# AdamClixby/Modulate

Measured on AMD Instinct MI355X. Metric: GB/s encrypt+decrypt over synthetic .ark parts; % HBM peak at 1/2/4/8 GPU, higher is better.
Workload: dtype u8

## Files before the change

include/modgpu_testing.h:

```cpp
#ifndef MODGPU_TESTING_H
#define MODGPU_TESTING_H

#include <stdint.h>

#ifdef __cplusplus
extern "C" {
#endif

int modgpu_time_cycle_device(void *dev_buf, uint64_t n, int32_t key, uint64_t stream_off,
                             int device, void *hip_stream, int iters, float *ms_per_launch);

int modgpu_time_cycle_device_to(void *dev_dst, const void *dev_src, uint64_t n, int32_t key, uint64_t stream_off,
                                int device, void *hip_stream, int iters, float *ms_per_launch);

int modgpu_time_rekey_device_to(void *dev_dst, const void *dev_src, uint64_t n, int32_t key_from, uint64_t off_from, int32_t key_to,
                                uint64_t off_to, int device, void *hip_stream, int iters, float *ms_per_launch);
int modgpu_time_cycle_table_device(const void *dev_entries, uint64_t n_entries, void *dev_workspace,
                                   uint64_t workspace_bytes, int device, void *hip_stream, int iters, float *ms_per_call);
int modgpu_time_rekey_table_device(const void *dev_entries, uint64_t n_entries, void *dev_workspace,
                                   uint64_t workspace_bytes, int device, void *hip_stream, int iters, float *ms_per_call);

int modgpu_time_verify_device(const void *dev_expect, const void *dev_src, uint64_t n, int32_t key, uint64_t stream_off,
                              void *dev_result, int device, void *hip_stream, int iters, float *ms_per_call);
int modgpu_time_digest_device(void *dev_dst, const void *dev_src, uint64_t n, int32_t key, uint64_t stream_off, void *dev_result,
// ... 53 lines not shown

int modgpu_cycle_scalar_host_isa(uint8_t *host_buf, uint64_t n, int32_t key, uint64_t stream_off, const char *isa);

int modgpu_numa_probe(const char *sysfs_root, const char *bdf, int *node, int *cpus, int max_cpus);

int modgpu_host_alloc_on_node(void **host_ptr, uint64_t n, int node);

void modgpu_queue_stats(uint64_t out[6]);

const char *modgpu_kernel_source_hash(void);
const char *modgpu_feed_kernel_source_hash(void);
const char *modgpu_to_kernel_source_hash(void);
const char *modgpu_xfer_kernel_source_hash(void);
const char *modgpu_rekey_kernel_source_hash(void);
const char *modgpu_table_kernel_source_hash(void);
const char *modgpu_rekey_table_kernel_source_hash(void);
const char *modgpu_verify_kernel_source_hash(void);
const char *modgpu_verify_table_kernel_source_hash(void);
const char *modgpu_rekey_verify_kernel_source_hash(void);
const char *modgpu_keep_kernel_source_hash(void);
const char *modgpu_rekey_verify_table_kernel_source_hash(void);
const char *modgpu_rekey_move_table_kernel_source_hash(void);
int modgpu_keep_policy(uint64_t bytes, uint32_t *mask, uint32_t *run);

int modgpu_testing_hooks(void);


void modgpu_debug_set_queue_ring(uint32_t lines);

void modgpu_debug_set_to_form(int form);

void modgpu_debug_set_rekey_form(int shape);

void modgpu_debug_set_table_grid(uint32_t grid);

void modgpu_debug_set_rekey_table_grid(uint32_t grid);

void modgpu_debug_set_move_grid(uint32_t grid);

void modgpu_debug_set_move_table_grid(uint32_t grid);

void modgpu_debug_set_verify_form(int grid);
void modgpu_debug_set_digest_grid(int grid);

void modgpu_debug_set_verify_table_grid(uint32_t grid);

void modgpu_debug_set_rekey_verify_table_grid(uint32_t grid);

void modgpu_debug_set_digest_table_grid(uint32_t grid);

void modgpu_debug_set_cycle_digest_table_grid(uint32_t grid);

void modgpu_debug_set_rekey_digest_table_grid(uint32_t grid);

void modgpu_debug_set_keep(uint64_t min_bytes, uint32_t mask, uint32_t run);

void modgpu_debug_set_xfer_form(int form);

void modgpu_debug_set_helpers(int mode);

void modgpu_debug_set_batch(int mode);

void modgpu_debug_set_launch(int variant, uint32_t grid_cap);

enum { MODGPU_TUNABLE_ZEROCOPY_BYTES = 0, MODGPU_TUNABLE_RING = 1, MODGPU_TUNABLE_SPLIT = 2, MODGPU_TUNABLE_CHUNK_MIN_BYTES = 3,
       MODGPU_TUNABLE_RAMP_BYTES = 4, MODGPU_TUNABLE_LANES = 5, MODGPU_TUNABLE_NTCOPY = 6,
       MODGPU_TUNABLE_FILE_SCHED = 7,
       MODGPU_TUNABLE_FEED = 8,
       MODGPU_TUNABLE_FEED_CHUNK_BYTES = 9,
       MODGPU_TUNABLE_FEED_PATIENCE_MS = 10,
       MODGPU_TUNABLE_FILE_FEED = 11,
       MODGPU_TUNABLE_XFER_LIST_MOST_BYTES = 12  };
void modgpu_debug_set_host_tunable(int which, uint64_t value);

void modgpu_debug_set_gpu_node(int node);

void modgpu_debug_set_pcie_grid(uint32_t cap);

// ... 22 lines not shown
```

modulate_amd/__init__.py:

```python
from .capi import (
    ModGpuError, lib, lib_path, device_count, cycle_host, cycle_device, hdr_decrypt_host,
    hdr_encrypt_host, cycle_parts_host, cycle_parts_device, cycle_batch_device, cycle_host_split, debug_set_batch, cycle_file, cycle_file_to_host, cycle_host_to_file, DeviceBuffer, time_cycle_device, state_at, jump_table,
    KEY_PS3, KEY_PS4, MAGIC_PS3, MAGIC_PS4, as_int32, EXPORTS, TESTING_EXPORTS, cycle_scalar_host, cycle_auto_host,
    path_stats, gpu_required, last_launch, debug_set_launch, debug_set_pinned_mode, debug_set_staged_mode, kernel_source_hash, feed_kernel_source_hash, prepare, host_tunables, debug_inject_failures, debug_inject_failure_at, debug_injection_armed, debug_hold_slots, debug_forbid_worker_threads, debug_set_pcie_grid, debug_set_gpu_node, debug_set_host_tunable, HOST_TUNABLES, STAGE_FILL, STAGE_LAUNCH, STAGE_SYNC, STAGE_DRAIN, STAGE_AFTER_DRAIN, STAGE_STALL, INJECT_PIECE_LAST, INJECT_PIECE_MIDDLE, PinnedBuffer, host_register, host_unregister,
    DEBUG_EXPORTS, FLAVOURS, testing_flavour, use_testing_flavour, active_flavour, debug_set_queue_ring, debug_set_helpers, queue_stats, testing_hooks, min_gpu_bytes,
    cycle_device_to, cycle_batch_device_to, time_cycle_device_to, to_kernel_source_hash, debug_set_to_form, TO_FORMS,
    rekey_device_to, rekey_batch_device_to, time_rekey_device_to, rekey_kernel_source_hash, debug_set_rekey_form, REKEY_FORMS,
    rekey_move_device, move_workspace_bytes, move_status, debug_set_move_grid,
    rekey_move_table_device, rekey_move_table_workspace_bytes, rekey_move_table_validate, rekey_move_table_status, compaction_table,
    rekey_move_table_kernel_source_hash, debug_set_move_table_grid,
    rekey_relayout_table_device, rekey_relayout_table_validate, relayout_table, splice_moves,
    cycle_table_device, time_cycle_table_device, table, table_workspace_bytes, table_status, table_validate, table_kernel_source_hash,
    debug_set_table_grid, TableEntry, TABLE_DTYPE,
    rekey_table_device, time_rekey_table_device, rekey_table, rekey_table_workspace_bytes, rekey_table_validate,
    rekey_table_kernel_source_hash, debug_set_rekey_table_grid, RekeyTableEntry, REKEY_TABLE_DTYPE,
    verify_device, verify_batch_device, verify_results, time_verify_device, verify_kernel_source_hash, debug_set_verify_form,
    VERIFY_RESULT_DTYPE, VERIFY_NONE,
    digest_device, digest_batch_device, digest_results, digest_adler32, time_digest_device, debug_set_digest_grid, DIGEST_RESULT_DTYPE,
    verify_table_device, verify_table_summary, verify_table_workspace_bytes, time_verify_table_device, verify_table_kernel_source_hash,
    debug_set_verify_table_grid, VERIFY_TABLE_SUMMARY_DTYPE,
    digest_table_device, digest_table_workspace_bytes, time_digest_table_device, debug_set_digest_table_grid,
    cycle_digest_table_device, cycle_digest_table_workspace_bytes, time_cycle_digest_table_device, debug_set_cycle_digest_table_grid,
    DIGEST_OUTPUT, DIGEST_INPUT,
    rekey_digest_table_device, rekey_digest_table_workspace_bytes, time_rekey_digest_table_device, debug_set_rekey_digest_table_grid,
    DIGEST_PLAIN,
    digest_check_device, digest_check_result, digest_check_bits_bytes, time_digest_check_device, DIGEST_CHECK_SUMMARY_DTYPE,
    verify_rekey_table_device, verify_rekey_table_workspace_bytes, time_verify_rekey_table_device, rekey_verify_table_kernel_source_hash,
    debug_set_rekey_verify_table_grid,
    verify_rekey_device, verify_rekey_batch_device, time_verify_rekey_device, rekey_verify_kernel_source_hash,
    keep_kernel_source_hash, keep_policy, debug_set_keep, KEEP_OFF,
    cycle_host_to_device, cycle_device_to_host, cycle_host_to_device_list, cycle_device_to_host_list, cycle_host_to_device_list_digest, cycle_device_to_host_list_digest, cycle_file_to_device, cycle_device_to_file, xfer_kernel_source_hash, debug_set_xfer_form, XFER_FORMS,
    host_loop_isa, cycle_scalar_host_isa, device_numa_node, numa_probe, host_policy, host_policy_engine, host_trace, host_trace_read, host_pool_stats, host_chunking, HOST_TRACE_KINDS,
)
```

modulate_amd/capi.py:

```python
import contextlib
import ctypes
import os

import numpy as np

_HERE = os.path.dirname(os.path.abspath(__file__))

KEY_PS3 = 0xC64EED30
KEY_PS4 = 0x90CFC0AB
MAGIC_PS3 = 0xC64EED30
MAGIC_PS4 = 0x6F303F55

_u64, _i32, _int, _vp = ctypes.c_uint64, ctypes.c_int32, ctypes.c_int, ctypes.c_void_p
EXPORTS = {
    "modgpu_abi_version": (_int, []),
    "modgpu_device_count": (_int, []),
    "modgpu_last_error": (ctypes.c_char_p, []),
    "modgpu_cycle_device": (_int, [_vp, _u64, _i32, _u64, _int, _vp]),
    "modgpu_cycle_host": (_int, [_vp, _u64, _i32, _u64, _int]),
    "modgpu_hdr_decrypt_host": (_int, [_vp, _u64, _int]),
    "modgpu_hdr_encrypt_host": (_int, [_vp, _u64, _int, _int]),
    "modgpu_cycle_parts_host": (_int, [ctypes.POINTER(_vp), ctypes.POINTER(_u64), _int, _i32, _int]),
    "modgpu_cycle_parts_device": (_int, [ctypes.POINTER(_vp), ctypes.POINTER(_u64), ctypes.POINTER(_int), _int, _i32]),
    "modgpu_cycle_host_split": (_int, [_vp, _u64, _i32, _u64, _int]),
# ... 150 lines not shown
    "modgpu_time_cycle_device_to": (_int, [_vp, _vp, _u64, _i32, _u64, _int, _vp, _int, ctypes.POINTER(ctypes.c_float)]),
    "modgpu_to_kernel_source_hash": (ctypes.c_char_p, []),
    "modgpu_xfer_kernel_source_hash": (ctypes.c_char_p, []),
    "modgpu_time_rekey_device_to": (_int, [_vp, _vp, _u64, _i32, _u64, _i32, _u64, _int, _vp, _int, ctypes.POINTER(ctypes.c_float)]),
    "modgpu_rekey_kernel_source_hash": (ctypes.c_char_p, []),
    "modgpu_time_cycle_table_device": (_int, [_vp, _u64, _vp, _u64, _int, _vp, _int, ctypes.POINTER(ctypes.c_float)]),
    "modgpu_table_kernel_source_hash": (ctypes.c_char_p, []),
    "modgpu_time_rekey_table_device": (_int, [_vp, _u64, _vp, _u64, _int, _vp, _int, ctypes.POINTER(ctypes.c_float)]),
    "modgpu_rekey_table_kernel_source_hash": (ctypes.c_char_p, []),
    "modgpu_time_verify_device": (_int, [_vp, _vp, _u64, _i32, _u64, _vp, _int, _vp, _int, ctypes.POINTER(ctypes.c_float)]),
    "modgpu_verify_kernel_source_hash": (ctypes.c_char_p, []),
    "modgpu_time_verify_table_device": (_int, [_vp, _u64, _vp, _vp, _u64, _int, _vp, _int, ctypes.POINTER(ctypes.c_float)]),
    "modgpu_verify_table_kernel_source_hash": (ctypes.c_char_p, []),
    "modgpu_time_digest_table_device": (_int, [_vp, _u64, _vp, _vp, _u64, _int, _vp, _int, ctypes.POINTER(ctypes.c_float)]),
    "modgpu_time_cycle_digest_table_device": (_int, [_vp, _u64, _vp, ctypes.c_uint32, _vp, _u64, _int, _vp, _int, ctypes.POINTER(ctypes.c_float)]),
    "modgpu_time_rekey_digest_table_device": (_int, [_vp, _u64, _vp, ctypes.c_uint32, _vp, _u64, _int, _vp, _int, ctypes.POINTER(ctypes.c_float)]),
    "modgpu_time_verify_rekey_device": (_int, [_vp, _vp, _u64, _i32, _u64, _i32, _u64, _vp, _int, _vp, _int, ctypes.POINTER(ctypes.c_float)]),
    "modgpu_rekey_verify_kernel_source_hash": (ctypes.c_char_p, []),
    "modgpu_keep_kernel_source_hash": (ctypes.c_char_p, []),
    "modgpu_time_verify_rekey_table_device": (_int, [_vp, _u64, _vp, _vp, _u64, _int, _vp, _int, ctypes.POINTER(ctypes.c_float)]),
    "modgpu_rekey_verify_table_kernel_source_hash": (ctypes.c_char_p, []),
    "modgpu_rekey_move_table_kernel_source_hash": (ctypes.c_char_p, []),
    "modgpu_keep_policy": (_int, [_u64, ctypes.POINTER(ctypes.c_uint32), ctypes.POINTER(ctypes.c_uint32)]),
    "modgpu_time_digest_device": (_int, [_vp, _vp, _u64, _i32, _u64, _vp, _int, _vp, _int, ctypes.POINTER(ctypes.c_float)]),
    "modgpu_time_digest_check_device": (_int, [_vp, _vp, _u64, _vp, _vp, _vp, _int, _vp, _int, ctypes.POINTER(ctypes.c_float)]),
}
DEBUG_EXPORTS = {
    "modgpu_debug_set_launch": (None, [_int, ctypes.c_uint32]),
    "modgpu_debug_set_pinned_mode": (None, [_int]),
    "modgpu_debug_set_staged_mode": (None, [_int]),
    "modgpu_debug_set_queue_ring": (None, [ctypes.c_uint32]),
    "modgpu_debug_set_helpers": (None, [_int]),
    "modgpu_debug_set_batch": (None, [_int]),
    "modgpu_debug_set_pcie_grid": (None, [ctypes.c_uint32]),
    "modgpu_debug_set_gpu_node": (None, [_int]),
    "modgpu_debug_set_host_tunable": (None, [_int, _u64]),
    "modgpu_debug_inject_failures": (None, [_int]),
    "modgpu_debug_inject_failure_at": (None, [ctypes.c_int64, _int]),
    "modgpu_debug_injection_armed": (_int, []),
    "modgpu_debug_hold_slots": (_int, [_int, _int]),
    "modgpu_debug_forbid_worker_threads": (None, [_int]),
    "modgpu_debug_set_to_form": (None, [_int]),
    "modgpu_debug_set_xfer_form": (None, [_int]),
    "modgpu_debug_set_rekey_form": (None, [_int]),
    "modgpu_debug_set_table_grid": (None, [ctypes.c_uint32]),
    "modgpu_debug_set_rekey_table_grid": (None, [ctypes.c_uint32]),
    "modgpu_debug_set_move_grid": (None, [ctypes.c_uint32]),
    "modgpu_debug_set_move_table_grid": (None, [ctypes.c_uint32]),
    "modgpu_debug_set_verify_form": (None, [_int]),
    "modgpu_debug_set_verify_table_grid": (None, [ctypes.c_uint32]),
    "modgpu_debug_set_rekey_verify_table_grid": (None, [ctypes.c_uint32]),
    "modgpu_debug_set_digest_table_grid": (None, [ctypes.c_uint32]),
    "modgpu_debug_set_cycle_digest_table_grid": (None, [ctypes.c_uint32]),
    "modgpu_debug_set_rekey_digest_table_grid": (None, [ctypes.c_uint32]),
    "modgpu_debug_set_keep": (None, [_u64, ctypes.c_uint32, ctypes.c_uint32]),
    "modgpu_debug_set_digest_grid": (None, [_int]),
}


class ModGpuError(RuntimeError):
    def __init__(self, code, text):
        super().__init__(f"modgpu error {code}: {text}")
        self.code = code


FLAVOURS = {"shipped": "libmodgpu.so", "testing": "libmodgpu_testing.so"}


def lib_path(flavour="shipped"):
    return os.environ.get("MODGPU_LIB") or os.path.join(_HERE, FLAVOURS[flavour])


_libs = {}
_active = "shipped"


def _load(flavour):
    if flavour not in _libs:
# ... 782 lines not shown

def time_verify_rekey_device(expect, src, n, key_from, key_to, result, off_from=0, off_to=0, device=-1, stream=None, iters=2):
    return _time_call("modgpu_time_verify_rekey_device", (_vp(_dev_addr(expect)), _vp(_dev_addr(src)), n, as_int32(key_from), off_from,
                                                          as_int32(key_to), off_to, _vp(_dev_addr(result))), device, stream, iters)


def keep_kernel_source_hash():
    return lib().modgpu_keep_kernel_source_hash().decode()


KEEP_OFF = (1 << 64) - 1


def keep_policy(nbytes):
    mask, run = ctypes.c_uint32(), ctypes.c_uint32()
    route = lib().modgpu_keep_policy(nbytes, ctypes.byref(mask), ctypes.byref(run))
    return bool(route), mask.value, run.value


def debug_set_keep(min_bytes=0, mask=0, run=0):
    _debug_lib().modgpu_debug_set_keep(min_bytes, mask, run)


def rekey_verify_kernel_source_hash():
    return lib().modgpu_rekey_verify_kernel_source_hash().decode()


def verify_table_workspace_bytes(n_entries):
    return lib().modgpu_verify_table_workspace_bytes(n_entries)


def verify_table_summary(workspace, device=-1):
    out = np.zeros(1, dtype=VERIFY_TABLE_SUMMARY_DTYPE)
    _check(lib().modgpu_verify_table_summary(_vp(_dev_addr(workspace)), device, _vp(out.ctypes.data)))
    first = int(out["first_bad_entry"][0])
    return {"mismatches": int(out["mismatches"][0]), "first_bad_entry": None if first == VERIFY_NONE else first, "entries": int(out["entries"][0])}


def verify_table_device(entries, results=None, workspace=None, device=-1, stream=None, *, n=None):
    return _table_call("modgpu_verify_table_device", entries, TABLE_DTYPE, n, workspace, verify_table_workspace_bytes, device, stream,
                       "the device refused verify table entry {}; no result was written", fetch=verify_results, results=results,
                       empty=_no_verify_results)


def time_verify_table_device(entries, n, results, workspace, device=-1, stream=None, iters=2):
    ws_bytes = workspace.nbytes if isinstance(workspace, DeviceBuffer) else verify_table_workspace_bytes(n)
# ... 470 lines not shown
```

modulate_amd/csrc/cycle_keep_kernel.h:

```cpp
#pragma once
#include <hip/hip_runtime.h>
#include <cstdint>

#include "cycle_kernel.h"

struct CycleKeepArgs : CycleQueueArgs {
    uint32_t keep_mask;
    uint32_t keep_run;
};
uint32_t modgpu_keep_chunk_bytes();
uint32_t modgpu_keep_block();
const char *modgpu_keep_kernel_name();
hipError_t modgpu_launch_cycle_keep(const CycleKeepArgs &a, uint32_t grid, hipStream_t stream);
```

modulate_amd/csrc/cycle_keep_kernel.hip:

```cpp
#include <hip/hip_runtime.h>
#include <cstdint>

#include "cycle_kernel_impl.h"
#include "cycle_keep_kernel.h"

#include <cstdio>

template <int U, int BLOCK>
__global__ __launch_bounds__(BLOCK) MODGPU_KEEP_OFF_THE_FIXED_TEMPORARIES void modgpu_cycle_keep_kernel(CycleKeepArgs a)
{
    static_assert(BLOCK % 256 == 0 && BLOCK <= 1024, "BLOCK is a whole number of 4096-byte tiles");
    constexpr int ALG = 2;
    constexpr int SAUX = AUX_SC1 | AUX_NT;
    constexpr int KAUX = AUX_SC1;
    constexpr int DEPTH = 1;
    constexpr uint32_t CHUNK = (uint32_t)U * BLOCK * lcg::WORD;
    constexpr uint32_t SUB = BLOCK * lcg::WORD;
    static_assert(CHUNK == 1u << 16, "the residency test reads the chunk's number off address bits 16 and up");
    constexpr int NB = DEPTH + 1;
    constexpr int PREFIX = DEPTH + 1;
    const uint32_t tid = threadIdx.x;
    const uint32_t blk = blockIdx.x;
    const uint32_t G = gridDim.x;
    const uint32_t Gm = a.main_groups != 0 && a.main_groups < G ? a.main_groups : G;
    const uint32_t n_parts = a.n_parts;
    const uint32_t total = a.start[kCycleBatchMax];
    __shared__ uint32_t q_next[2];
    uint32_t trip = 0;
    const uint32_t voff = tid * lcg::WORD;
    const uint32_t lane_mul = mulmod_canon(c_tile_lo.v[tid >> 8], c_lane_pow.v[tid & 255]);

    for (uint32_t p = blk; p < n_parts; p += G) {
        const CycleQueuePart &P = a.part[p];
        const uint64_t body_bytes = P.end - P.lead;
        if (tid < 32) cycle_edges(P.body - P.head_n, P.head_n, P.base_head, P.body + body_bytes, P.tail_n, P.base_tail, tid);
        if (P.lead != 0 && body_bytes != 0) {
            const uint64_t inside = P.end < CHUNK ? body_bytes : CHUNK - P.lead;
            auto r = __builtin_amdgcn_make_buffer_rsrc(P.body, 0, (int)inside, 0x00020000);
            uint32_t su = mulmod_canon(P.base_body, lane_mul);
#pragma unroll 1
            for (uint32_t u = 0; u < (uint32_t)U; ++u) {
                const uint32_t o = voff + u * SUB - P.lead;
                u32x4 d = __builtin_amdgcn_raw_buffer_load_b128(r, o, 0, AUX_NT);
                d = cycle_word<ALG>(d, su);
                __builtin_amdgcn_raw_buffer_store_b128(d, r, o, 0, SAUX);
                su = mulmod_canon(su, lcg::kTileLo.v[BLOCK / 256]);
            }
        }
    }
// ... 11 lines not shown
#pragma unroll 1
        for (uint32_t i = 1; i < n_parts; ++i) p += g >= a.start[i] ? 1u : 0u;
        const CycleQueuePart &P = a.part[p];
        v.origin = P.body - P.lead;
        v.end = P.end;
        v.first = P.lead != 0 ? 1u : 0u;
        v.lo = a.start[p];
        v.hi = a.start[p + 1];
        v.lane_base = mulmod_canon(P.base_body, lane_mul);
    };
    auto rsrc_at = [&](uint32_t g, const View &v) {
        const uint64_t o = (uint64_t)(v.first + (g - v.lo)) * CHUNK;
        const uint64_t left = g < v.hi && o < v.end ? v.end - o : 0;
        return __builtin_amdgcn_make_buffer_rsrc(v.origin + o, 0, (int)(left < CHUNK ? left : CHUNK), 0x00020000);
    };
    auto states = [&](uint32_t g, const View &v, uint32_t(&s)[U]) {
        const uint32_t c = v.first + (g - v.lo);
        uint32_t p = mulmod_canon(c_chunk_pow0<CHUNK>.v[c & 255], c_chunk_pow1<CHUNK>.v[(c >> 8) & 255]);
        p = mulmod_canon(p, c_chunk_pow2<CHUNK>.v[(c >> 16) & 255]);
        s[0] = mulmod_canon(v.lane_base, p);
#pragma unroll
        for (int u = 1; u < U; ++u) s[u] = mulmod_canon(s[u - 1], lcg::kTileLo.v[BLOCK / 256]);
    };
    View vl{nullptr, 0, 0, 0, 0, 1}, vs{nullptr, 0, 0, 0, 0, 1};
    auto load = [&](u32x4(&d)[U], uint32_t g) {
        locate(g, vl);
        auto r = rsrc_at(g, vl);
#pragma unroll
        for (int u = 0; u < U; ++u) d[u] = __builtin_amdgcn_raw_buffer_load_b128(r, voff + u * SUB, 0, AUX_NT);
    };
    uint32_t pending = 0;
    const uint32_t q_next_lds = (uint32_t)(uintptr_t)(__attribute__((address_space(3))) uint32_t *)&q_next[0];
    const uint32_t one = 1u;
    auto process_store = [&](u32x4(&d)[U], uint32_t g) {
        locate(g, vs);
        auto r = rsrc_at(g, vs);
        const uint64_t addr = (uint64_t)reinterpret_cast<uintptr_t>(vs.origin) + (uint64_t)(vs.first + (g - vs.lo)) * CHUNK;
        const bool resident = ((uint32_t)(addr >> 16) & a.keep_mask) < a.keep_run;
        uint32_t s[U];
        states(g, vs, s);
#pragma unroll
        for (int u = 0; u < U; ++u) d[u] = cycle_word<ALG>(d[u], s[u]);
        if (tid == 0)
            asm volatile("ds_write_b32 %0, %1\n\ts_waitcnt lgkmcnt(0)" : : "v"(q_next_lds + 4u * (trip & 1u)), "v"(pending) : "memory");
        __builtin_amdgcn_sched_barrier(0);
        __builtin_amdgcn_s_barrier();
        if (resident) {
#pragma unroll
            for (int u = 0; u < U; ++u) __builtin_amdgcn_raw_buffer_store_b128(d[u], r, voff + u * SUB, 0, KAUX);
        } else {
#pragma unroll
            for (int u = 0; u < U; ++u) __builtin_amdgcn_raw_buffer_store_b128(d[u], r, voff + u * SUB, 0, SAUX);
        }
        ++trip;
    };
    auto take_published = [&]() {
        uint32_t t;
        asm volatile("ds_read_b32 %0, %1\n\ts_waitcnt lgkmcnt(0)" : "=v"(t) : "v"(q_next_lds + 4u * ((trip - 1u) & 1u)) : "memory");
        return (uint32_t)PREFIX * Gm + (uint32_t)__builtin_amdgcn_readfirstlane((int)t);
    };

    uint32_t cq[NB];
    static_assert(PREFIX == NB, "the static positions are exactly the ones cq[] starts with");
    bool active = true;
    if (blk < Gm) {
#pragma unroll
        for (int i = 0; i < NB; ++i) cq[i] = blk + (uint32_t)i * Gm;
    } else {
        uint32_t t = 0xFFFFFFFFu;
        if (tid == 0) {
            const uint64_t t0 = wall_clock64(), c0 = clock64();
            uint64_t t1;
            do {
                __builtin_amdgcn_s_sleep(4);
                t1 = wall_clock64();
            } while (t1 - t0 < 200);
            const uint64_t mhz = ((clock64() - c0) * 100) / (t1 - t0);
            if (mhz < a.helper_below_mhz) t = __hip_atomic_fetch_add(a.queue, (uint32_t)PREFIX, __ATOMIC_RELAXED, __HIP_MEMORY_SCOPE_AGENT);
            q_next[0] = t;
        }
        __syncthreads();
        t = q_next[0];
        __syncthreads();
        active = t != 0xFFFFFFFFu;
#pragma unroll
        for (int i = 0; i < NB; ++i) cq[i] = (uint32_t)PREFIX * Gm + t + (uint32_t)i;
    }
    if (active && cq[0] < total) {
        u32x4 d[NB][U];
#pragma unroll
        for (int i = 0; i < DEPTH; ++i) load(d[i], cq[i]);
        bool finished = false;
        while (!finished) {
#pragma unroll
            for (int p = 0; p < NB; ++p) {
                __builtin_amdgcn_s_barrier();
                if (tid == 0) pending = __hip_atomic_fetch_add(a.queue, one, __ATOMIC_RELAXED, __HIP_MEMORY_SCOPE_AGENT);
                load(d[(p + DEPTH) % NB], cq[DEPTH]);
                __builtin_amdgcn_sched_barrier(0);
                process_store(d[p], cq[0]);
#pragma unroll
                for (int i = 0; i < DEPTH; ++i) cq[i] = cq[i + 1];
                cq[DEPTH] = take_published();
                if (cq[0] >= total) {
                    finished = true;
                    break;
                }
            }
        }
    }
    if (tid == 0) {
        asm volatile("s_waitcnt vmcnt(0)" ::: "memory");
        if (atomicAdd(a.queue + 1, 1u) == G - 1) {
            __hip_atomic_store(a.queue, 0u, __ATOMIC_RELAXED, __HIP_MEMORY_SCOPE_AGENT);
            __hip_atomic_store(a.queue + 1, 0u, __ATOMIC_RELAXED, __HIP_MEMORY_SCOPE_AGENT);
            if (a.queue_done) {
                asm volatile("s_waitcnt vmcnt(0)" ::: "memory");
                __hip_atomic_store(a.queue_done, a.queue_seq, __ATOMIC_RELAXED, __HIP_MEMORY_SCOPE_SYSTEM);
            }
        }
    }
}

namespace {
template <int U, int BLOCK> struct KeepShape {
    static constexpr uint32_t chunk = (uint32_t)U * BLOCK * lcg::WORD;
    static constexpr uint32_t block = BLOCK;
    static void launch(const CycleKeepArgs &a, uint32_t grid, hipStream_t stream)
    {
        hipLaunchKernelGGL((modgpu_cycle_keep_kernel<U, BLOCK>), dim3(grid), dim3(BLOCK), 0, stream, a);
    }
    static const char *name()
    {
        static char buf[96];
        static const int n = std::snprintf(buf, sizeof buf, "modgpu_cycle_keep_kernel<%d, %d>", U, BLOCK);
        (void)n;
        return buf;
    }
// ... 13 lines not shown
```

modulate_amd/csrc/modgpu_capi.cpp:

```cpp
#include <hip/hip_runtime.h>

#include <algorithm>
#include <cctype>
#include <cerrno>
#include <cstdlib>
#include <cstring>
#include <mutex>
#include <thread>
#include <vector>

#include "../../include/modgpu_testing.h"
#include "crossover_table.h"
#include "cycle_feed_kernel.h"
#include "cycle_keep_kernel.h"
#include "cycle_kernel.h"
#include "cycle_rekey_kernel.h"
#include "cycle_rekey_table_kernel.h"
#include "cycle_rekey_move_table_kernel.h"
#include "cycle_verify_table_kernel.h"
#include "cycle_rekey_verify_table_kernel.h"
#include "cycle_verify_kernel.h"
#include "cycle_rekey_verify_kernel.h"
#include "cycle_table_kernel.h"
#include "cycle_to_kernel.h"
// ... 165 lines not shown
{
    if ((device >= 0 || always_save) && hipGetDevice(&prev_) != hipSuccess) {
        (void)hipGetLastError();
        prev_ = -1;
    }
    rc = device >= 0 || !always_save ? select_device(device) : MODGPU_OK;
}

DeviceScope::~DeviceScope()
{
    if (prev_ >= 0) (void)hipSetDevice(prev_);
}


namespace {

struct Plan {
    CycleArgs args;
    int variant;
    uint32_t grid;
};

thread_local modgpu_launch_info_t t_last_launch{};
#ifdef MODGPU_TESTING_HOOKS
std::atomic<int> g_force_variant{-1};
std::atomic<uint32_t> g_grid_cap{0};
std::atomic<uint32_t> g_pcie_grid{0};
int forced_variant() { return g_force_variant.load(std::memory_order_relaxed); }
uint32_t forced_grid_cap() { return g_grid_cap.load(std::memory_order_relaxed); }
uint32_t forced_pcie_grid() { return g_pcie_grid.load(std::memory_order_relaxed); }
#else
constexpr int forced_variant() { return -1; }
constexpr uint32_t forced_grid_cap() { return 0; }
constexpr uint32_t forced_pcie_grid() { return 0; }
#endif

uint32_t large_grid()
{
    static std::mutex mu;
    static uint32_t cus[kMaxDevices] = {};
    int dev = 0;
    if (hipGetDevice(&dev) != hipSuccess || dev < 0 || dev >= kMaxDevices) return 256u;
    std::lock_guard<std::mutex> lock(mu);
    if (!cus[dev]) {
        int n = 0;
        if (hipDeviceGetAttribute(&n, hipDeviceAttributeMultiprocessorCount, dev) != hipSuccess || n <= 0) n = 256;
// ... 137 lines not shown
    return by_dev[dev];
}
#ifdef MODGPU_TESTING_HOOKS
std::atomic<int> g_helper_mode{0};
int helper_mode() { return g_helper_mode.load(std::memory_order_relaxed); }
#else
constexpr int helper_mode() { return 0; }
#endif

#ifdef MODGPU_TESTING_HOOKS
std::atomic<int> g_batch_mode{0};
int batch_mode() { return g_batch_mode.load(std::memory_order_relaxed); }
#else
constexpr int batch_mode() { return 0; }
#endif
std::atomic<uint64_t> g_batch_launches{0}, g_batch_parts{0};

constexpr uint32_t kSmallGridMax = 16384u;
constexpr uint64_t kLargeMin = (256ull << 20) + 1;

constexpr uint64_t kKeepMin = 1ull << 30;
constexpr uint64_t kKeepBytes = 192ull << 20;
constexpr uint32_t kKeepMask = 255u;
struct KeepPolicy {
    bool route;
    uint32_t mask, run;
};
#ifdef MODGPU_TESTING_HOOKS
std::mutex g_keep_mutex;
uint64_t g_keep_min = 0;
uint32_t g_keep_mask = 0, g_keep_run = 0;
#endif
KeepPolicy keep_policy(uint64_t bytes)
{
#ifdef MODGPU_TESTING_HOOKS
    {
        std::lock_guard<std::mutex> lock(g_keep_mutex);
        if (g_keep_min != 0) return {bytes >= g_keep_min, g_keep_mask, g_keep_run};
    }
#endif
    if (bytes < kKeepMin) return {false, kKeepMask, 0u};
    return {true, kKeepMask, (uint32_t)std::min<uint64_t>(kKeepBytes * (kKeepMask + 1ull) / bytes, kKeepMask + 1ull)};
}

constexpr uint32_t kPcieGridMax = 256u;
constexpr uint32_t kPcieGridShort = 32u;
constexpr uint64_t kPcieShortMax = 64ull << 20;

void queue_grid(uint64_t chunks, uint64_t cus, uint64_t *main_cap, uint64_t *helpers)
{
    const uint32_t grid_cap = forced_grid_cap();
    uint64_t cap = std::max<uint64_t>(1, cus * 25 / 32);
    const bool capped = grid_cap >= 1 && grid_cap < cus;
    if (capped && grid_cap < cap) cap = grid_cap;
    *helpers = 0;
    if (helper_mode() == 1) *helpers = capped ? std::max<uint64_t>(1, cap * 7 / 25) : cus - cap;
    else if (helper_mode() == 0 && !capped && chunks >= 4 * cus) *helpers = cus - cap;
    *main_cap = cap;
}

int choose_variant(const void *dev_buf, uint64_t n, bool over_pcie)
{
    const int forced = forced_variant();
    if (forced >= 0 && forced < kCycleVariants) return forced;
    const uint64_t head = std::min<uint64_t>(n, (16 - (reinterpret_cast<uintptr_t>(dev_buf) & 15)) & 15);
// ... 57 lines not shown
        P.base_tail = lcg::state_residue(key_res, o + head + (words * 16) % lcg::PERIOD);
        const uint64_t n_chunks = (P.end + chunk - 1) / chunk, first = P.lead != 0 ? 1 : 0;
        if (n_chunks >= (1ull << 24)) return 1;
        a.start[k] = (uint32_t)total;
        total += n_chunks > first ? n_chunks - first : 0;
        bytes += sizes[k];
    }
    for (int k = n; k <= kCycleBatchMax; ++k) a.start[k] = (uint32_t)total;
    a.n_parts = (uint32_t)n;
    const QueuePair q = queue_pair(stream);
    if (!q.pair) return 1;
    a.queue = q.pair;
    a.queue_done = q.done;
    a.queue_seq = q.seq;
    uint64_t cap = 0, helpers = 0;
    queue_grid(total, large_grid(), &cap, &helpers);
    const uint64_t main_groups = std::max<uint64_t>(1, std::min<uint64_t>(total, cap));
    a.main_groups = (uint32_t)main_groups;
    a.helper_below_mhz = helper_mode() == 1 ? 0xFFFFFFFFu : helper_below_mhz();
    const uint32_t grid = (uint32_t)(main_groups + helpers);
    const KeepPolicy keep = n != 1 ? KeepPolicy{false, 0u, 0u} : warm_keep ? KeepPolicy{true, kKeepMask, 0u} : keep_policy(bytes);
    hipError_t e;
    if (keep.route) {
        CycleKeepArgs ka{};
        static_cast<CycleQueueArgs &>(ka) = a;
        ka.keep_mask = keep.mask;
        ka.keep_run = keep.run;
        e = modgpu_launch_cycle_keep(ka, grid, stream);
    } else {
        e = modgpu_launch_cycle_queue(a, grid, stream);
    }
    if (e != hipSuccess) {
        queue_pair_unused(q);
        return fail_hip(e, "cycle kernel launch (work queue)");
    }
    g_stats.gpu_launches.fetch_add(1, std::memory_order_relaxed);
    if (n > 1) {
        g_batch_launches.fetch_add(1, std::memory_order_relaxed);
        g_batch_parts.fetch_add((uint64_t)n, std::memory_order_relaxed);
    }
    if (keep.route) t_last_launch = {modgpu_keep_kernel_name(), CYCLE_QUEUE, grid, modgpu_keep_block(), (uint32_t)chunk, bytes, (uint32_t)main_groups, MODGPU_KEEP_KERNEL_SOURCE_HASH};
    else t_last_launch = {modgpu_queue_kernel_name(), n > 1 ? CYCLE_BATCH : CYCLE_QUEUE, grid, modgpu_queue_block(), (uint32_t)chunk, bytes, (uint32_t)main_groups, MODGPU_KERNEL_SOURCE_HASH};
    return MODGPU_OK;
}

}

int cycle_device_impl(void *dev_buf, uint64_t n, int32_t key, uint64_t stream_off, hipStream_t stream, bool over_pcie)
{
    if (n == 0) return MODGPU_OK;
// ... 2260 lines not shown

const char *modgpu_kernel_source_hash(void) { return MODGPU_KERNEL_SOURCE_HASH; }
const char *modgpu_feed_kernel_source_hash(void) { return MODGPU_FEED_KERNEL_SOURCE_HASH; }
const char *modgpu_to_kernel_source_hash(void) { return MODGPU_TO_KERNEL_SOURCE_HASH; }
const char *modgpu_xfer_kernel_source_hash(void) { return MODGPU_XFER_KERNEL_SOURCE_HASH; }
const char *modgpu_rekey_kernel_source_hash(void) { return MODGPU_REKEY_KERNEL_SOURCE_HASH; }
const char *modgpu_table_kernel_source_hash(void) { return MODGPU_TABLE_KERNEL_SOURCE_HASH; }
const char *modgpu_rekey_table_kernel_source_hash(void) { return MODGPU_REKEY_TABLE_KERNEL_SOURCE_HASH; }
const char *modgpu_verify_kernel_source_hash(void) { return MODGPU_VERIFY_KERNEL_SOURCE_HASH; }
const char *modgpu_verify_table_kernel_source_hash(void) { return MODGPU_VERIFY_TABLE_KERNEL_SOURCE_HASH; }
const char *modgpu_rekey_verify_kernel_source_hash(void) { return MODGPU_REKEY_VERIFY_KERNEL_SOURCE_HASH; }
const char *modgpu_keep_kernel_source_hash(void) { return MODGPU_KEEP_KERNEL_SOURCE_HASH; }
const char *modgpu_rekey_verify_table_kernel_source_hash(void) { return MODGPU_REKEY_VERIFY_TABLE_KERNEL_SOURCE_HASH; }
const char *modgpu_rekey_move_table_kernel_source_hash(void) { return MODGPU_REKEY_MOVE_TABLE_KERNEL_SOURCE_HASH; }

int modgpu_keep_policy(uint64_t bytes, uint32_t *mask, uint32_t *run)
{
    const KeepPolicy k = keep_policy(bytes);
    if (mask) *mask = k.mask;
    if (run) *run = k.run;
    return k.route ? 1 : 0;
}

int modgpu_time_cycle_table_device(const void *dev_entries, uint64_t n_entries, void *dev_workspace, uint64_t workspace_bytes,
                                   int device, void *hip_stream, int iters, float *ms_per_call)
{
    return guarded([&]() -> int {
        return time_calls(device, hip_stream, iters, ms_per_call, [&](hipStream_t st) {
            return table_impl(static_cast<const modgpu_table_entry_t *>(dev_entries), n_entries, nullptr, 0u, dev_workspace, workspace_bytes, -1, st);
        });
    });
}

int modgpu_time_cycle_digest_table_device(const void *dev_entries, uint64_t n_entries, void *dev_records, uint32_t side, void *dev_workspace,
                                          uint64_t workspace_bytes, int device, void *hip_stream, int iters, float *ms_per_call)
{
    return guarded([&]() -> int {
        return time_calls(device, hip_stream, iters, ms_per_call, [&](hipStream_t st) {
            return cycle_digest_table_impl(static_cast<const modgpu_table_entry_t *>(dev_entries), n_entries, static_cast<modgpu_digest_result_t *>(dev_records), side, dev_workspace, workspace_bytes, -1, st);
        });
    });
}

int modgpu_time_rekey_table_device(const void *dev_entries, uint64_t n_entries, void *dev_workspace, uint64_t workspace_bytes,
                                   int device, void *hip_stream, int iters, float *ms_per_call)
{
// ... 90 lines not shown
void modgpu_debug_set_table_grid(uint32_t grid) { force_table_grid(kCycleTable, grid); }
void modgpu_debug_set_move_grid(uint32_t grid) { g_move_grid.store(std::min<uint32_t>(grid, 4096u), std::memory_order_relaxed); }
void modgpu_debug_set_move_table_grid(uint32_t grid) { force_table_grid(kMoveTable, grid); }
void modgpu_debug_set_rekey_table_grid(uint32_t grid) { force_table_grid(kRekeyTable, grid); }
void modgpu_debug_set_rekey_digest_table_grid(uint32_t grid) { force_table_grid(kRekeyDigestTable, grid); }

void modgpu_debug_set_verify_table_grid(uint32_t grid) { force_table_grid(kVerifyTable, grid); }
void modgpu_debug_set_rekey_verify_table_grid(uint32_t grid) { force_table_grid(kRekeyVerifyTable, grid); }
void modgpu_debug_set_digest_table_grid(uint32_t grid) { force_table_grid(kDigestTable, grid); }
void modgpu_debug_set_cycle_digest_table_grid(uint32_t grid) { force_table_grid(kCycleDigestTable, grid); }

void modgpu_debug_set_verify_form(int grid) { g_verify_grid.store(grid <= 0 ? 0u : std::min<uint32_t>((uint32_t)grid, 4096u), std::memory_order_relaxed); }

void modgpu_debug_set_digest_grid(int grid) { g_digest_grid.store(grid <= 0 ? 0u : std::min<uint32_t>((uint32_t)grid, 4096u), std::memory_order_relaxed); }

void modgpu_debug_set_keep(uint64_t min_bytes, uint32_t mask, uint32_t run)
{
    std::lock_guard<std::mutex> lock(g_keep_mutex);
    g_keep_min = min_bytes;
    g_keep_mask = min_bytes ? mask : 0u;
    g_keep_run = min_bytes ? run : 0u;
}

void modgpu_debug_set_queue_ring(uint32_t lines)
{
    g_ring_lines.store(lines == 0 ? kQueueRing : std::min(lines, kQueueRing), std::memory_order_relaxed);
}
#endif

}
```

Baseline: 3555.

## Split keep-kernel chunk queue into main and resident lanes by address rank

Replaces the keep kernel's single linear chunk queue with two address-derived lanes: main chunks and cache-resident chunks. Each lane is mapped through rank/unrank arithmetic with a precomputed reciprocal, and a second queue counter serves the resident lane. A configurable slice of helper groups can be dedicated to the resident lane so residency-friendly chunks are drained separately from streaming chunks. The default slice permille is zero, so by default lane_run is cleared and all chunks flow through the main lane, but the new indexing math now runs per chunk. A debug hook and query API are added to inspect and force the slice.

```diff
diff --git a/include/modgpu_testing.h b/include/modgpu_testing.h
--- a/include/modgpu_testing.h
+++ b/include/modgpu_testing.h
@@ -99,6 +99,7 @@
 const char *modgpu_rekey_verify_table_kernel_source_hash(void);
 const char *modgpu_rekey_move_table_kernel_source_hash(void);
 int modgpu_keep_policy(uint64_t bytes, uint32_t *mask, uint32_t *run);
+int modgpu_keep_slice(const void *dev_buf, uint64_t bytes, uint32_t main_groups, uint32_t helpers, uint32_t out[4]);
 
 int modgpu_testing_hooks(void);
 
@@ -131,6 +132,8 @@
 void modgpu_debug_set_rekey_digest_table_grid(uint32_t grid);
 
 void modgpu_debug_set_keep(uint64_t min_bytes, uint32_t mask, uint32_t run);
+
+void modgpu_debug_set_keep_slice(int groups);
 
 void modgpu_debug_set_xfer_form(int form);
 
diff --git a/modulate_amd/__init__.py b/modulate_amd/__init__.py
--- a/modulate_amd/__init__.py
+++ b/modulate_amd/__init__.py
@@ -28,7 +28,7 @@
     verify_rekey_table_device, verify_rekey_table_workspace_bytes, time_verify_rekey_table_device, rekey_verify_table_kernel_source_hash,
     debug_set_rekey_verify_table_grid,
     verify_rekey_device, verify_rekey_batch_device, time_verify_rekey_device, rekey_verify_kernel_source_hash,
-    keep_kernel_source_hash, keep_policy, debug_set_keep, KEEP_OFF,
+    keep_kernel_source_hash, keep_policy, debug_set_keep, KEEP_OFF, keep_slice, debug_set_keep_slice,
     cycle_host_to_device, cycle_device_to_host, cycle_host_to_device_list, cycle_device_to_host_list, cycle_host_to_device_list_digest, cycle_device_to_host_list_digest, cycle_file_to_device, cycle_device_to_file, xfer_kernel_source_hash, debug_set_xfer_form, XFER_FORMS,
     host_loop_isa, cycle_scalar_host_isa, device_numa_node, numa_probe, host_policy, host_policy_engine, host_trace, host_trace_read, host_pool_stats, host_chunking, HOST_TRACE_KINDS,
 )
diff --git a/modulate_amd/capi.py b/modulate_amd/capi.py
--- a/modulate_amd/capi.py
+++ b/modulate_amd/capi.py
@@ -196,6 +196,7 @@
     "modgpu_rekey_verify_table_kernel_source_hash": (ctypes.c_char_p, []),
     "modgpu_rekey_move_table_kernel_source_hash": (ctypes.c_char_p, []),
     "modgpu_keep_policy": (_int, [_u64, ctypes.POINTER(ctypes.c_uint32), ctypes.POINTER(ctypes.c_uint32)]),
+    "modgpu_keep_slice": (_int, [ctypes.c_void_p, _u64, ctypes.c_uint32, ctypes.c_uint32, ctypes.POINTER(ctypes.c_uint32)]),
     "modgpu_time_digest_device": (_int, [_vp, _vp, _u64, _i32, _u64, _vp, _int, _vp, _int, ctypes.POINTER(ctypes.c_float)]),
     "modgpu_time_digest_check_device": (_int, [_vp, _vp, _u64, _vp, _vp, _vp, _int, _vp, _int, ctypes.POINTER(ctypes.c_float)]),
 }
@@ -228,6 +229,7 @@
     "modgpu_debug_set_cycle_digest_table_grid": (None, [ctypes.c_uint32]),
     "modgpu_debug_set_rekey_digest_table_grid": (None, [ctypes.c_uint32]),
     "modgpu_debug_set_keep": (None, [_u64, ctypes.c_uint32, ctypes.c_uint32]),
+    "modgpu_debug_set_keep_slice": (None, [_int]),
     "modgpu_debug_set_digest_grid": (None, [_int]),
 }
 
@@ -1056,6 +1058,16 @@
     _debug_lib().modgpu_debug_set_keep(min_bytes, mask, run)
 
 
+def keep_slice(ptr=None, nbytes=0, main_groups=0, helpers=0):
+    out = (ctypes.c_uint32 * 4)()
+    route = lib().modgpu_keep_slice(ctypes.c_void_p(int(getattr(ptr, "ptr", ptr)) if ptr is not None else None), nbytes, main_groups, helpers, out)
+    return {"route": bool(route), "n_main": out[0], "n_res": out[1], "slice_groups": out[2], "k_permille": out[3]}
+
+
+def debug_set_keep_slice(groups=-1):
+    _debug_lib().modgpu_debug_set_keep_slice(groups)
+
+
 def rekey_verify_kernel_source_hash():
     return lib().modgpu_rekey_verify_kernel_source_hash().decode()
 
diff --git a/modulate_amd/csrc/cycle_keep_kernel.h b/modulate_amd/csrc/cycle_keep_kernel.h
--- a/modulate_amd/csrc/cycle_keep_kernel.h
+++ b/modulate_amd/csrc/cycle_keep_kernel.h
@@ -7,7 +7,89 @@
 struct CycleKeepArgs : CycleQueueArgs {
     uint32_t keep_mask;
     uint32_t keep_run;
+    uint32_t keep_shift;
+    uint32_t slice_groups;
+    uint32_t n_main, n_res;
+    uint32_t main_off, res_off;
+    uint32_t lane_run;
+    uint32_t inv_main, inv_res;
 };
+
+#if defined(__HIPCC__)
+#define MODGPU_KEEP_MAP __host__ __device__ inline
+#else
+#define MODGPU_KEEP_MAP inline
+#endif
+
+MODGPU_KEEP_MAP uint32_t keep_rank_res(uint32_t y, uint32_t mask, uint32_t run, uint32_t shift)
+{
+    const uint32_t in = y & mask;
+    return (mask == 0xFFFFFFFFu ? 0u : (y >> shift) * run) + (in < run ? in : run);
+}
+MODGPU_KEEP_MAP uint32_t keep_rank_main(uint32_t y, uint32_t mask, uint32_t run, uint32_t shift)
+{
+    return y - keep_rank_res(y, mask, run, shift);
+}
+MODGPU_KEEP_MAP uint32_t keep_per_period_res(uint32_t run) { return run ? run : 1u; }
+MODGPU_KEEP_MAP uint32_t keep_per_period_main(uint32_t mask, uint32_t run)
+{
+    const uint64_t n = (uint64_t)mask + 1u - run;
+    return n == 0 ? 1u : n > 0xFFFFFFFFull ? 0xFFFFFFFFu : (uint32_t)n;
+}
+MODGPU_KEEP_MAP uint32_t keep_inverse(uint32_t per) { return per > 1u ? (uint32_t)((1ull << 32) / per) : 0xFFFFFFFFu; }
+MODGPU_KEEP_MAP uint32_t keep_div(uint32_t j, uint32_t per, uint32_t inv)
+{
+    const uint32_t q = (uint32_t)(((uint64_t)j * inv) >> 32);
+    return q + (j - q * per >= per ? 1u : 0u);
+}
+MODGPU_KEEP_MAP uint32_t keep_unrank(uint32_t j, uint32_t per, uint32_t inv, uint32_t shift, uint32_t first_in_period)
+{
+    const uint32_t q = keep_div(j, per, inv);
+    return (q << shift) + first_in_period + (j - q * per);
+}
+MODGPU_KEEP_MAP uint32_t keep_unrank_res(uint32_t j, uint32_t mask, uint32_t run, uint32_t shift)
+{
+    return keep_unrank(j, keep_per_period_res(run), keep_inverse(keep_per_period_res(run)), shift, 0u);
+}
+MODGPU_KEEP_MAP uint32_t keep_unrank_main(uint32_t j, uint32_t mask, uint32_t run, uint32_t shift)
+{
+    return keep_unrank(j, keep_per_period_main(mask, run), keep_inverse(keep_per_period_main(mask, run)), shift, run);
+}
+
+MODGPU_KEEP_MAP bool keep_plan_lanes(CycleKeepArgs &a, uint64_t x0, uint32_t total)
+{
+    const uint32_t mask = a.keep_mask, run = a.lane_run;
+    uint32_t shift = 0;
+    while (shift < 31 && (mask >> shift) != 0) ++shift;
+    const uint32_t y0 = (uint32_t)x0 & mask;
+    if ((uint64_t)y0 + total > 0xFFFFFFFFull) return false;
+    a.keep_shift = shift;
+    a.res_off = keep_rank_res(y0, mask, run, shift);
+    a.main_off = y0 - a.res_off;
+    a.n_res = keep_rank_res(y0 + total, mask, run, shift) - a.res_off;
+    a.n_main = total - a.n_res;
+    a.inv_main = keep_inverse(keep_per_period_main(mask, run));
+    a.inv_res = keep_inverse(keep_per_period_res(run));
+    return true;
+}
+constexpr uint32_t KEEP_SKIP = 0xFFFFFFFEu, KEEP_DONE = 0xFFFFFFFFu;
+struct KeepLane {
+    uint32_t word, lim, add, per, inv, fip;
+};
+MODGPU_KEEP_MAP KeepLane keep_lane_main(const CycleKeepArgs &a, uint32_t drawn)
+{
+    return KeepLane{0u, a.n_main > drawn ? a.n_main - drawn : 0u, drawn + a.main_off, keep_per_period_main(a.keep_mask, a.lane_run), a.inv_main,
+                    a.lane_run - (a.main_off + a.res_off)};
+}
+MODGPU_KEEP_MAP KeepLane keep_lane_res(const CycleKeepArgs &a)
+{
+    return KeepLane{2u, a.n_res, a.res_off, keep_per_period_res(a.lane_run), a.inv_res, 0u - (a.main_off + a.res_off)};
+}
+MODGPU_KEEP_MAP uint32_t keep_lane_chunk(const KeepLane &L, uint32_t shift, uint32_t t)
+{
+    return t < L.lim ? keep_unrank(t + L.add, L.per, L.inv, shift, L.fip) : L.word ? KEEP_DONE : KEEP_SKIP;
+}
+
 uint32_t modgpu_keep_chunk_bytes();
 uint32_t modgpu_keep_block();
 const char *modgpu_keep_kernel_name();
diff --git a/modulate_amd/csrc/cycle_keep_kernel.hip b/modulate_amd/csrc/cycle_keep_kernel.hip
--- a/modulate_amd/csrc/cycle_keep_kernel.hip
+++ b/modulate_amd/csrc/cycle_keep_kernel.hip
@@ -25,6 +25,7 @@
     const uint32_t Gm = a.main_groups != 0 && a.main_groups < G ? a.main_groups : G;
     const uint32_t n_parts = a.n_parts;
     const uint32_t total = a.start[kCycleBatchMax];
+    constexpr uint32_t SKIP = KEEP_SKIP, DONE = KEEP_DONE;
     __shared__ uint32_t q_next[2];
     uint32_t trip = 0;
     const uint32_t voff = tid * lcg::WORD;
@@ -82,10 +83,10 @@
 #pragma unroll
         for (int u = 1; u < U; ++u) s[u] = mulmod_canon(s[u - 1], lcg::kTileLo.v[BLOCK / 256]);
     };
-    View vl{nullptr, 0, 0, 0, 0, 1}, vs{nullptr, 0, 0, 0, 0, 1};
+    View vs{nullptr, 0, 0, 0, 0, 1};
     auto load = [&](u32x4(&d)[U], uint32_t g) {
-        locate(g, vl);
-        auto r = rsrc_at(g, vl);
+        locate(g, vs);
+        auto r = rsrc_at(g, vs);
 #pragma unroll
         for (int u = 0; u < U; ++u) d[u] = __builtin_amdgcn_raw_buffer_load_b128(r, voff + u * SUB, 0, AUX_NT);
     };
@@ -117,26 +118,35 @@
     auto take_published = [&]() {
         uint32_t t;
         asm volatile("ds_read_b32 %0, %1\n\ts_waitcnt lgkmcnt(0)" : "=v"(t) : "v"(q_next_lds + 4u * ((trip - 1u) & 1u)) : "memory");
-        return (uint32_t)PREFIX * Gm + (uint32_t)__builtin_amdgcn_readfirstlane((int)t);
-    };
+        return (uint32_t)__builtin_amdgcn_readfirstlane((int)t);
+    };
+    auto chunk_at = [&](const KeepLane &L, uint32_t t) { return keep_lane_chunk(L, a.keep_shift, t); };
 
     uint32_t cq[NB];
     static_assert(PREFIX == NB, "the static positions are exactly the ones cq[] starts with");
     bool active = true;
+    KeepLane L = keep_lane_main(a, (uint32_t)PREFIX * Gm);
     if (blk < Gm) {
-#pragma unroll
-        for (int i = 0; i < NB; ++i) cq[i] = blk + (uint32_t)i * Gm;
+        const KeepLane S = keep_lane_main(a, 0u);
+#pragma unroll
+        for (int i = 0; i < NB; ++i) cq[i] = chunk_at(S, blk + (uint32_t)i * Gm);
     } else {
+        const bool slice = blk - Gm < a.slice_groups;
+        if (slice) L = keep_lane_res(a);
         uint32_t t = 0xFFFFFFFFu;
         if (tid == 0) {
-            const uint64_t t0 = wall_clock64(), c0 = clock64();
-            uint64_t t1;
-            do {
-                __builtin_amdgcn_s_sleep(4);
-                t1 = wall_clock64();
-            } while (t1 - t0 < 200);
-            const uint64_t mhz = ((clock64() - c0) * 100) / (t1 - t0);
-            if (mhz < a.helper_below_mhz) t = __hip_atomic_fetch_add(a.queue, (uint32_t)PREFIX, __ATOMIC_RELAXED, __HIP_MEMORY_SCOPE_AGENT);
+            bool join = slice;
+            if (!slice) {
+                const uint64_t t0 = wall_clock64(), c0 = clock64();
+                uint64_t t1;
+                do {
+                    __builtin_amdgcn_s_sleep(4);
+                    t1 = wall_clock64();
+                } while (t1 - t0 < 200);
+                const uint64_t mhz = ((clock64() - c0) * 100) / (t1 - t0);
+                join = mhz < a.helper_below_mhz;
+            }
+            if (join) t = __hip_atomic_fetch_add(a.queue + L.word, (uint32_t)PREFIX, __ATOMIC_RELAXED, __HIP_MEMORY_SCOPE_AGENT);
             q_next[0] = t;
         }
         __syncthreads();
@@ -144,9 +154,10 @@
         __syncthreads();
         active = t != 0xFFFFFFFFu;
 #pragma unroll
-        for (int i = 0; i < NB; ++i) cq[i] = (uint32_t)PREFIX * Gm + t + (uint32_t)i;
-    }
-    if (active && cq[0] < total) {
+        for (int i = 0; i < NB; ++i) cq[i] = chunk_at(L, t + (uint32_t)i);
+    }
+    if (cq[DEPTH] == SKIP) L = keep_lane_res(a);
+    if (active && (cq[0] < total || (cq[0] == SKIP && a.n_res != 0))) {
         u32x4 d[NB][U];
 #pragma unroll
         for (int i = 0; i < DEPTH; ++i) load(d[i], cq[i]);
@@ -155,14 +166,15 @@
 #pragma unroll
             for (int p = 0; p < NB; ++p) {
                 __builtin_amdgcn_s_barrier();
-                if (tid == 0) pending = __hip_atomic_fetch_add(a.queue, one, __ATOMIC_RELAXED, __HIP_MEMORY_SCOPE_AGENT);
+                if (tid == 0) pending = __hip_atomic_fetch_add(a.queue + L.word, one, __ATOMIC_RELAXED, __HIP_MEMORY_SCOPE_AGENT);
                 load(d[(p + DEPTH) % NB], cq[DEPTH]);
                 __builtin_amdgcn_sched_barrier(0);
                 process_store(d[p], cq[0]);
 #pragma unroll
                 for (int i = 0; i < DEPTH; ++i) cq[i] = cq[i + 1];
-                cq[DEPTH] = take_published();
-                if (cq[0] >= total) {
+                cq[DEPTH] = chunk_at(L, take_published());
+                if (cq[DEPTH] == SKIP) L = keep_lane_res(a);
+                if (cq[0] >= SKIP && cq[DEPTH] == DONE) {
                     finished = true;
                     break;
                 }
@@ -174,6 +186,7 @@
         if (atomicAdd(a.queue + 1, 1u) == G - 1) {
             __hip_atomic_store(a.queue, 0u, __ATOMIC_RELAXED, __HIP_MEMORY_SCOPE_AGENT);
             __hip_atomic_store(a.queue + 1, 0u, __ATOMIC_RELAXED, __HIP_MEMORY_SCOPE_AGENT);
+            __hip_atomic_store(a.queue + 2, 0u, __ATOMIC_RELAXED, __HIP_MEMORY_SCOPE_AGENT);
             if (a.queue_done) {
                 asm volatile("s_waitcnt vmcnt(0)" ::: "memory");
                 __hip_atomic_store(a.queue_done, a.queue_seq, __ATOMIC_RELAXED, __HIP_MEMORY_SCOPE_SYSTEM);
diff --git a/modulate_amd/csrc/modgpu_capi.cpp b/modulate_amd/csrc/modgpu_capi.cpp
--- a/modulate_amd/csrc/modgpu_capi.cpp
+++ b/modulate_amd/csrc/modgpu_capi.cpp
@@ -211,6 +211,7 @@
 };
 
 thread_local modgpu_launch_info_t t_last_launch{};
+thread_local uint32_t t_last_keep[3] = {};
 #ifdef MODGPU_TESTING_HOOKS
 std::atomic<int> g_force_variant{-1};
 std::atomic<uint32_t> g_grid_cap{0};
@@ -394,6 +395,7 @@
 constexpr uint64_t kKeepMin = 1ull << 30;
 constexpr uint64_t kKeepBytes = 192ull << 20;
 constexpr uint32_t kKeepMask = 255u;
+constexpr uint32_t kKeepSlicePermille = 0;
 struct KeepPolicy {
     bool route;
     uint32_t mask, run;
@@ -402,6 +404,10 @@
 std::mutex g_keep_mutex;
 uint64_t g_keep_min = 0;
 uint32_t g_keep_mask = 0, g_keep_run = 0;
+std::atomic<int> g_keep_slice{-1};
+int forced_keep_slice() { return g_keep_slice.load(std::memory_order_relaxed); }
+#else
+constexpr int forced_keep_slice() { return -1; }
 #endif
 KeepPolicy keep_policy(uint64_t bytes)
 {
@@ -413,6 +419,34 @@
 #endif
     if (bytes < kKeepMin) return {false, kKeepMask, 0u};
     return {true, kKeepMask, (uint32_t)std::min<uint64_t>(kKeepBytes * (kKeepMask + 1ull) / bytes, kKeepMask + 1ull)};
+}
+
+uint32_t keep_slice_rule(uint64_t main_groups, uint64_t helpers, uint64_t n_main, uint64_t n_res, uint32_t permille)
+{
+    if (!helpers || !n_res || !permille) return 0u;
+    if (!n_main) return (uint32_t)helpers;
+    return (uint32_t)std::min<uint64_t>(helpers, (permille * main_groups * n_res + 1000u * n_main - 1u) / (1000u * n_main));
+}
+
+void keep_lanes(CycleKeepArgs &ka, const KeepPolicy &keep, uintptr_t chunk0, uint32_t total, uint64_t main_groups, uint64_t helpers, uint32_t *by_address = nullptr)
+{
+    const bool pattern = (keep.mask & (keep.mask + 1u)) == 0u;
+    ka.keep_mask = pattern ? keep.mask : 0u;
+    ka.keep_run = pattern ? (uint32_t)std::min<uint64_t>(keep.run, (uint64_t)keep.mask + 1u) : 0u;
+    ka.lane_run = ka.keep_run;
+    if (!keep_plan_lanes(ka, (uint64_t)chunk0 >> 16, total)) {
+        ka.keep_mask = ka.keep_run = ka.lane_run = 0u;
+        (void)keep_plan_lanes(ka, (uint64_t)chunk0 >> 16, total);
+    }
+    if (by_address) by_address[0] = ka.n_main, by_address[1] = ka.n_res;
+    const int forced = forced_keep_slice();
+    ka.slice_groups = !ka.n_res    ? 0u
+                      : forced >= 0 ? (uint32_t)std::min<uint64_t>(helpers, (uint64_t)forced)
+                                    : keep_slice_rule(main_groups, helpers, ka.n_main, ka.n_res, kKeepSlicePermille);
+    if (forced < 0 && ka.slice_groups == 0u && ka.lane_run != 0u) {
+        ka.lane_run = 0u;
+        (void)keep_plan_lanes(ka, (uint64_t)chunk0 >> 16, total);
+    }
 }
 
 constexpr uint32_t kPcieGridMax = 256u;
@@ -516,10 +550,12 @@
     const KeepPolicy keep = n != 1 ? KeepPolicy{false, 0u, 0u} : warm_keep ? KeepPolicy{true, kKeepMask, 0u} : keep_policy(bytes);
     hipError_t e;
     if (keep.route) {
+        static_assert(sizeof(uintptr_t) == 8, "a chunk's number is its 64-bit address >> 16");
         CycleKeepArgs ka{};
         static_cast<CycleQueueArgs &>(ka) = a;
-        ka.keep_mask = keep.mask;
-        ka.keep_run = keep.run;
+        const CycleQueuePart &P = a.part[0];
+        keep_lanes(ka, keep, reinterpret_cast<uintptr_t>(P.body) - P.lead + (P.lead != 0 ? chunk : 0), (uint32_t)total, main_groups, helpers);
+        t_last_keep[0] = ka.n_main, t_last_keep[1] = ka.n_res, t_last_keep[2] = ka.slice_groups;
         e = modgpu_launch_cycle_keep(ka, grid, stream);
     } else {
         e = modgpu_launch_cycle_queue(a, grid, stream);
@@ -2826,6 +2862,27 @@
     return k.route ? 1 : 0;
 }
 
+int modgpu_keep_slice(const void *dev_buf, uint64_t bytes, uint32_t main_groups, uint32_t helpers, uint32_t out[4])
+{
+    if (!out) return 0;
+    out[3] = kKeepSlicePermille;
+    if (!dev_buf) {
+        out[0] = t_last_keep[0], out[1] = t_last_keep[1], out[2] = t_last_keep[2];
+        return 1;
+    }
+    const uint64_t chunk = modgpu_keep_chunk_bytes();
+    const uintptr_t addr = reinterpret_cast<uintptr_t>(dev_buf);
+    const uint64_t head = std::min<uint64_t>(bytes, (16 - (addr & 15)) & 15), words = (bytes - head) / 16;
+    const uint64_t lead = (addr + head) & (chunk - 1), n_chunks = (lead + words * 16 + chunk - 1) / chunk, first = lead != 0 ? 1 : 0;
+    const KeepPolicy k = keep_policy(bytes);
+    out[0] = out[1] = out[2] = 0;
+    if (n_chunks >= (1ull << 24)) return 0;
+    CycleKeepArgs ka{};
+    keep_lanes(ka, k, addr + head - lead + first * chunk, (uint32_t)(n_chunks > first ? n_chunks - first : 0), main_groups, helpers, out);
+    out[2] = ka.slice_groups;
+    return k.route ? 1 : 0;
+}
+
 int modgpu_time_cycle_table_device(const void *dev_entries, uint64_t n_entries, void *dev_workspace, uint64_t workspace_bytes,
                                    int device, void *hip_stream, int iters, float *ms_per_call)
 {
@@ -2962,6 +3019,8 @@
     g_keep_run = min_bytes ? run : 0u;
 }
 
+void modgpu_debug_set_keep_slice(int groups) { g_keep_slice.store(groups < 0 ? -1 : groups, std::memory_order_relaxed); }
+
 void modgpu_debug_set_queue_ring(uint32_t lines)
 {
     g_ring_lines.store(lines == 0 ? kQueueRing : std::min(lines, kQueueRing), std::memory_order_relaxed);
```

Result: no change. 3545 (-0.3%).
